# NILOIDE/A.I.gar

Hardware: AMD Instinct MI355X
Metric: env-steps/sec at 4096 bots x 100k pellets; 1/2/4/8 MI355X scaling (higher is better)
Workload: dtype f64; 1 GPU; C3: 4096 bots, 100000 pellets, 1152 viruses, split p=0.0025, eject p=0.01, field 4800, obs 854 floats/bot; start: data/c3_t50.npz (tick 50, mean cell mass 17.45, max 51.3) + 30 untimed random-policy ticks to settle; policy=random, parallelism=single-gpu

## Files before the change

aigar_amd/csrc/aigar_dev.h:

```cpp
#pragma once
#include <stdint.h>

#include "../../include/aigar.h"

namespace aigar {

#ifdef AIGAR_FLOOR
#ifdef AIGAR_FLOOR_OPAQUE
#define FLOOR(k) \
  if ((((AIGAR_FLOOR) >> (k)) & 1) && d.A > 0) return
#else
#define FLOOR(k) \
  if (((AIGAR_FLOOR) >> (k)) & 1) return
#endif
#else
#define FLOOR(k)
#endif

struct ArenaCtl {
  int64_t seq_next;
  int64_t tick;
  int64_t tick_sp;
  uint64_t key0, key1, ctr_pellet, ctr_virus;
  int64_t seq_base_upd;
// ... 31 lines not shown
  uint32_t pl_epoch;
  int pl_ticket;
  int n_pel_glob, n_eaten_glob, n_out, n_out_pel, n_undone, n_undone_glob;
  int n_ho;
  int n_ho_live;
  int n_cmd;
  int64_t stat[8];
};

enum : uint32_t {
  ERR_PELLET_CAP = 1, ERR_BLOB_CAP = 2, ERR_VIRUS_CAP = 4, ERR_EVENT_CAP = 8, ERR_WORK_CAP = 16,
  ERR_OBS_CAP = 32, ERR_CAND_CAP = 64, ERR_SLOT = 128, ERR_PIX_CAP = 256, ERR_TILE_CAP = 512, ERR_TILE_LOOKUP = 1024,
  ERR_TILE_OBS = 2048,
  ERR_TILE_PASSES = 4096,
  ERR_PREDICT = 8192,
  ERR_TILE_HANDOFF = 16384,
  ERR_CLAIM = 32768
};
enum : uint32_t { WARN_NEW_VIRUS_EATS = 1, WARN_DEAD_VIRUS = 2, WARN_TILE_OBS = 4 };
enum : uint32_t { DIRTY_VIRUS = 1, DIRTY_BLOB = 2 };

enum : uint32_t { PH_MERGE = 0, PH_VB = 1, PH_PV = 2, PH_PELLET = 3, PH_BLOB = 4, PH_PP = 5, PH_SPAWN = 6 };

struct TileRec {
  int32_t kind, idx;
  int64_t seq;
  double x, y;
};
enum : int32_t { TR_HDR = 0, TR_PELLET = 1, TR_BLOB = 2, TR_CELL = 3, TR_HIST = 4, TR_CMD = 5 };
constexpr int kHcapMax = 256;

struct alignas(32) PelRec {
// ... 38 lines not shown
  double *spec_x, *spec_y, *spec_m;
  double pow_n032[17];
  int cshift;
  int cshift_c;
  int Pcap, Ecap, Vcap, Wcap, EVcap;
  int PR;
  int PS;
  int PD;
  int PH1;
  int virus_enabled;
  double max_pellets, max_viruses;
  int G, L;
  uint32_t obs_ch, obs_ex;
  int flags;
  int pp_par;
  int share_cells;
  ArenaCtl *ctl;
  int *p_alive, *p_respawn, *p_ncells, *p_split, *p_eject, *p_pend;
  double *p_cmdx, *p_cmdy;
  double *p_fx, *p_fy, *p_fs, *p_mass;
  int *p_split_lh;
  uint8_t *p_role;
  int *p_time;
  double *o_last_mass;
  uint8_t *p_list;
  int *p_newc, *p_newb, *p_seqoff, *p_bloboff;
  int *p_heavy;
  double *c_x, *c_y, *c_m, *c_r, *c_vx, *c_vy, *c_svx, *c_svy, *c_mt;
  int *c_svc;
  uint32_t *c_flags;
  int64_t *c_seq;
// ... 70 lines not shown
```

aigar_amd/csrc/api.hip:

```cpp
#include <dlfcn.h>
#include <hip/hip_runtime.h>

#include <algorithm>
#include <cmath>
#include <cstdarg>
#include <cstdio>
#include <cstdlib>
#include <cstring>
#include <string>
#include <vector>

#include "../../include/aigar.h"
#include "aigar_dev.h"
#include "aigar_sem.h"

namespace aigar {
void launch_tick(const Dev &d, hipStream_t s, int rounds, int64_t *scr_k, int *scr_v,
                 const RandomPolicy *rp = nullptr);
void launch_tick_pre(const Dev &d, hipStream_t s, int64_t *scr_k, int *scr_v, const RandomPolicy *rp);
void launch_tick_post(const Dev &d, hipStream_t s, int64_t *scr_k, int *scr_v);
void launch_tile_pass(const Dev &d, hipStream_t s, int rounds, int64_t *scr_k, int *scr_v, int first);
void launch_tile_policy(const Dev &d, hipStream_t s, int greedy_split, uint8_t *mask, int cap);
void launch_tile_cmd_apply(const Dev &d, hipStream_t s, int box_recs);
void launch_pel_gather(const Dev &d, hipStream_t s, int a);
// ... 265 lines not shown
      cfg->obs_channels & (AIGAR_OBS_SELF_LF | AIGAR_OBS_SELF_SLF | AIGAR_OBS_ENEMY_LF | AIGAR_OBS_ENEMY_SLF))
    return fail("aigar_create: ALL_PLAYER_GRID with last-frame grids is undefined in the reference");
  if ((cfg->flags & AIGAR_FLAG_SCORE) &&
      (std::max(1, cfg->tile_x) * std::max(1, cfg->tile_y) > 1 || (cfg->tile_flags & AIGAR_TILE_FORCE)))
    return fail("aigar_create: AIGAR_FLAG_SCORE (the mass history score) is not kept on a tiled handle");
  int ndev = 0;
  HIPCHK(hipGetDeviceCount(&ndev));
  if (cfg->device < 0 || cfg->device >= ndev) return fail("aigar_create: device %d not present (%d devices)", cfg->device, ndev);
  HIPCHK(hipSetDevice(cfg->device));
  aigar_handle *h = new aigar_handle();
  h->cfg = *cfg;
  if (getenv("AIGAR_NO_GRAPH")) h->use_graph = false;
  if (const char *u = getenv("AIGAR_RUN_UNROLL")) h->run_unroll = std::max(1, std::min(64, atoi(u)));
  if (getenv("AIGAR_TILE_GRAPH")) h->tile_graph = true;
  h->d.pp_par = getenv("AIGAR_PP_SERIAL") ? 0 : 1;
  h->d.share_cells = 0;
  if (const char *r = getenv("AIGAR_FOOD_ROUNDS")) h->rounds = std::max(1, std::min(16, atoi(r)));
  Dev &d = h->d;
  d.A = cfg->n_arenas;
  d.B = cfg->bots_per_arena;
  d.NP = d.A * d.B;
  d.size = cfg->field_size > 0 ? cfg->field_size : (int)(75 * std::sqrt((double)d.B));
  d.cols = (int)std::ceil(d.size / 20.0);
  d.H = d.cols * d.cols;
  d.virus_enabled = cfg->virus_enabled ? 1 : 0;
  d.max_pellets = cfg->max_pellets >= 0 ? cfg->max_pellets : (double)d.size * d.size * 0.015;
  d.max_viruses = cfg->max_viruses >= 0 ? cfg->max_viruses : (double)d.size * d.size * 0.00005;
  if (!d.virus_enabled) d.max_viruses = 0;
  auto r64 = [](int v) { return (v + 63) / 64 * 64; };
  d.Ecap = r64(cfg->blob_cap > 0 ? cfg->blob_cap : 4 * d.B + 256);
  d.Pcap = r64(cfg->pellet_cap > 0 ? cfg->pellet_cap : (int)std::ceil(d.max_pellets) + d.Ecap + 64);
// ... 207 lines not shown
  free_all(h);
  delete h;
  return 0;
}

static int check_device_errors(aigar_handle *h) {
  std::vector<ArenaCtl> ctl(h->d.A);
  HIPCHK(hipMemcpyAsync(ctl.data(), h->d.ctl, sizeof(ArenaCtl) * h->d.A, hipMemcpyDeviceToHost, h->stream));
  HIPCHK(hipStreamSynchronize(h->stream));
  for (int a = 0; a < h->d.A; a++)
    if (ctl[a].err)
      return fail("device error bits 0x%x in arena %d (1 pellet cap, 2 blob cap, 4 virus cap, 8 event cap, "
                  "16 worklist cap, 32 observation cap, 64 candidate cap, 128 slot, 256 pixel-frame object cap, "
                  "512 tile message cap, 1024 tile record lookup, 2048 tile view beyond the held pellets, "
                  "4096 tiled tick ended with undone cells, 8192 new-cell / blob counts not as predicted, "
                  "16384 more dead bots to hand off than hand-off slots, 32768 cell claims left at the claim bound)",
                  ctl[a].err, a);
  return 0;
}

static size_t pix_hist_bytes(const aigar_handle *h) {
  return (h->pix.flags & AIGAR_PIX_LAST) ? sizeof(uint32_t) * h->d.NP * (size_t)h->pix.side * h->pix.side : 0;
}
__global__ void __launch_bounds__(256) k_pix_hist_clear_arenas(uint32_t *hist, size_t row, const int *al) {
  uint32_t *p = hist + (size_t)al[blockIdx.y] * row;
  for (size_t i = blockIdx.x * (size_t)blockDim.x + threadIdx.x; i < row; i += (size_t)gridDim.x * blockDim.x) p[i] = 0;
}
__global__ void __launch_bounds__(256) k_pix_hist_clear_bots(uint32_t *hist, size_t LL, size_t n, const uint8_t *mask) {
  const size_t i = blockIdx.x * (size_t)blockDim.x + threadIdx.x;
  if (i < n && (!mask || mask[i / LL])) hist[i] = 0;
}
// ... 159 lines not shown
    else launch_tick(h->d, h->stream, rounds, h->scr_k, h->scr_v);
  }
  HIPCHK(hipGetLastError());
  return 0;
}

static void launch_env_step(aigar_handle *h, hipStream_t s, const aigar_run_params &p, void *out, int dtype,
                            bool policy_done = false, bool fuse_next = false) {
#ifdef AIGAR_NO_POLICY_FOLD
  const RandomPolicy rp{0, 0, 0, 0};
  if (p.policy == AIGAR_POLICY_RANDOM) launch_policy(h->d, s, p.p_split, p.p_eject, p.seed);
#else
  const RandomPolicy rp{p.policy == AIGAR_POLICY_RANDOM, p.p_split, p.p_eject, p.seed};
#endif
  if (p.policy == AIGAR_POLICY_GREEDY && !policy_done) launch_policy_greedy(h->d, s, p.greedy_split ? 1 : 0, nullptr, -1);
  Dev dt = h->d;
  dt.share_cells = p.policy == AIGAR_POLICY_GREEDY ? 1 : 0;
  launch_tick(dt, s, food_rounds(h), h->scr_k, h->scr_v, &rp);
  if (out) launch_observe(h->d, s, out, dtype, 0, nullptr, fuse_next ? (p.greedy_split ? 1 : 0) : -1);
}
static bool run_fuses_greedy(const aigar_handle *h, const aigar_run_params &p, const void *out) {
  return p.policy == AIGAR_POLICY_GREEDY && out && observe_fuses_greedy(h->d) &&
         !getenv("AIGAR_NO_GREEDY_FUSE");
}

extern "C" int aigar_run(aigar_handle *h, int n_steps, const aigar_run_params *p, void *obs_out, int dtype) {
  if (!h || !p) return fail("null argument");
  if (n_steps < 0) return fail("n_steps < 0");
  if (p->policy < AIGAR_POLICY_NONE || p->policy > AIGAR_POLICY_GREEDY) return fail("unknown policy %d", p->policy);
  if (obs_out && dtype != 0 && dtype != 1) return fail("dtype must be 0 (float64) or 1 (float32)");
  HIPCHK(hipSetDevice(h->cfg.device));
  if (h->d.flags & AIGAR_FLAG_EVENTS)
    hipLaunchKernelGGL(k_step_begin, dim3((h->d.A + 63) / 64), dim3(64), 0, h->stream, h->d);
// ... 1325 lines not shown
```

aigar_amd/csrc/tick.hip:

```cpp
#include <hip/hip_runtime.h>

#include "aigar_dev.h"
#include "aigar_sem.h"
#include "aigar_wave.h"

namespace aigar {

#define GTID ((int)(blockIdx.x * blockDim.x + threadIdx.x))
#define TILE_GATE(d)                                          \
  do {                                                        \
    if ((d).tile_gate && (d).ctl[0].n_undone_glob == 0) return; \
  } while (0)

#ifdef AIGAR_PHASE_TIMING
constexpr int kPtWaves = 8192;
__device__ unsigned int g_ptw[9][kPtWaves][8];
__device__ unsigned int g_ptid[9][kPtWaves][2];
__device__ __forceinline__ void pt_ids(unsigned *o) {
  unsigned a, b;
  asm volatile("s_getreg_b32 %0, hwreg(HW_REG_HW_ID)" : "=s"(a));
  asm volatile("s_getreg_b32 %0, hwreg(HW_REG_XCC_ID)" : "=s"(b));
  o[0] = a;
  o[1] = b;
}
// ... 1233 lines not shown
  __syncthreads();
}
__device__ __forceinline__ int cgrid_cols(const Dev &d) { return (d.cols + (1 << d.cshift_c) - 1) >> d.cshift_c; }
__device__ __forceinline__ int cgrid_bucket(const Dev &d, double x, double y) {
  const int sh = d.cshift_c;
  return (center_bucket_coord(y, d.cols) >> sh) * cgrid_cols(d) + (center_bucket_coord(x, d.cols) >> sh);
}
__device__ __forceinline__ int *cgrid_counts(const Dev &d, int a, int row) {
  return d.cgcnt + ((size_t)a * 2 + row) * CG_STRIDE;
}
__device__ __forceinline__ void cgrid_count_cell(const Dev &d, int a, size_t ci, double x, double y) {
  const int per = kMaxCells * d.B, slot = (int)(ci / d.NP), p = (int)(ci - (size_t)slot * d.NP) - a * d.B;
  const int b = cgrid_bucket(d, x, y);
  d.c_rank[(size_t)a * per + (size_t)slot * d.B + p] = (b << 17) | atomicAdd(&cgrid_counts(d, a, 0)[b], 1);
}
__device__ void count_scan_256(int *cnt, int n, int *start, int *lds, uint16_t *bits) {
  __shared__ int wsum[4];
  const int tid = threadIdx.x, lane = tid & 63, w = tid >> 6;
  const int4 *c4 = reinterpret_cast<const int4 *>(cnt);
  int v[16], sum = 0;
#pragma unroll
  for (int k = 0; k < 4; k++) {
    const int j = tid * 16 + 4 * k;
    int4 q = j < n ? c4[j >> 2] : make_int4(0, 0, 0, 0);
    v[4 * k] = j < n ? q.x : 0;
    v[4 * k + 1] = j + 1 < n ? q.y : 0;
    v[4 * k + 2] = j + 2 < n ? q.z : 0;
    v[4 * k + 3] = j + 3 < n ? q.w : 0;
  }
#pragma unroll
  for (int k = 0; k < 16; k++) sum += v[k];
  if (bits) {
    uint32_t bm = 0;
#pragma unroll
    for (int k = 0; k < 16; k++) bm |= (v[k] != 0 ? 1u : 0u) << k;
    bits[tid] = (uint16_t)bm;
  }
  int inc = sum;
#pragma unroll
  for (int off = 1; off < 64; off <<= 1) {
    int t = __shfl_up(inc, off);
    if (lane >= off) inc += t;
  }
  if (lane == 63) wsum[w] = inc;
  __syncthreads();
  int run = inc - sum;
  for (int k = 0; k < w; k++) run += wsum[k];
  const int total = wsum[0] + wsum[1] + wsum[2] + wsum[3];
#pragma unroll
  for (int k = 0; k < 16; k++) {
    const int j = tid * 16 + k;
    if (j < n) {
      start[j] = run;
      if (lds) lds[j] = run;
      cnt[j] = 0;
    }
    run += v[k];
  }
  if (tid == 0) {
    start[n] = total;
    if (lds) lds[n] = total;
  }
}
__device__ void cgrid_scan_block(const Dev &d, int a) {
  const int cc = cgrid_cols(d);
  count_scan_256(cgrid_counts(d, a, 0), cc * cc, d.cstart + (size_t)a * (d.H + 1), nullptr, nullptr);
}
__device__ __forceinline__ void cgrid_place_player(const Dev &d, int gp, int n) {
  const int NP = d.NP, a = gp / d.B, p = gp - a * d.B, per = kMaxCells * d.B;
  const int *start = d.cstart + (size_t)a * (d.H + 1);
  int *items = d.citems + (size_t)a * per;
  for (int k = 0; k < n; k++) {
    const int slot = d.p_list[k * NP + gp];
    const int br = d.c_rank[(size_t)a * per + (size_t)slot * d.B + p];
    items[start[br >> 17] + (br & 0x1FFFF)] = slot * NP + gp;
  }
}


__device__ __forceinline__ int prow_entry(const Dev &d, int bx, int by) { return by * (d.cols + 1) + bx; }
__device__ __forceinline__ void prow_count(const Dev &d, int a, int j) {
// ... 195 lines not shown
  const int *st = d.vstart + (size_t)a * (d.H + 1);
  const int *it = d.vitems + (size_t)a * d.Vcap;
  const int nv = c.n_vir;
  grid_visit(st, it, d.cols, qb, expand_for(c.rmax_virus), [&](int i) {
    const size_t g = (size_t)a * d.Vcap + i;
    if (i >= nv || !(d.v_flags[g] & F_ALIVE)) return;
    const double vx = d.v_x[g], vy = d.v_y[g], vr = d.v_r[g];
    if (!rect_hit(footprint(vx, vy, vr, d.size), qb)) return;
    if (!overlap(vx, vy, d.v_m[g], vr, bx, by, bm, br)) return;
    if (atomicExch(&d.v_active[g], 1) != 0) return;
    const int w = atomicAdd(&d.ctl[a].n_pend, 1);
    if (w < d.Wcap) d.work[(size_t)a * d.Wcap + w] = i;
    else set_err(d, a, ERR_WORK_CAP);
  }, d.cshift);
}
__device__ void count_scan_256(int *cnt, int n, int *start, int *lds, uint16_t *bits);
__device__ void blob_grid_place(const Dev &d, int a, int *cnt) {
  const int tid = threadIdx.x, T = blockDim.x, s = d.cshift;
  const int cc = (d.cols + (1 << s) - 1) >> s;
  const int n = d.ctl[a].n_blob;
  int *items = d.bitems + (size_t)a * d.Ecap;
  const int *rank = d.b_rank + (size_t)a * d.Ecap;
  count_scan_256(cgrid_counts(d, a, 1), cc * cc, d.bstart + (size_t)a * (d.H + 1), cnt,
                 reinterpret_cast<uint16_t *>(d.bmap + (size_t)a * 64));
  __syncthreads();
  if (tid == 0) d.ctl[a].n_blob_live = cnt[cc * cc];
  for (int i = tid; i < n; i += T) {
    const int rk = rank[i];
    if (rk < 0) continue;
    const int b = rk >> 12, r = rk & 4095;
    if (r == 4095) set_err(d, a, ERR_SLOT);
// ... 475 lines not shown

__device__ __forceinline__ void wave_sync_lds() {
  __builtin_amdgcn_fence(__ATOMIC_RELEASE, "wavefront");
  __builtin_amdgcn_wave_barrier();
  __builtin_amdgcn_fence(__ATOMIC_ACQUIRE, "wavefront");
}
__device__ __forceinline__ double wave_sum(double v) {
#pragma unroll
  for (int off = 32; off > 0; off >>= 1) v += __shfl_xor(v, off);
  return v;
}

constexpr int PREP_CAND = 128;
constexpr int PREP_WAVES = 1;
__device__ __forceinline__ double tile_rall() { return sqrt(kMaxMass / kPi) * (1 + 1e-9); }
template <bool SHARE>
__global__ void __launch_bounds__(256, 4) k_food_prep(Dev d, int rounds, int resume) {
  FLOOR(4);
  TILE_GATE(d);
  __shared__ int64_t s_seq[4][PREP_CAND];
  __shared__ double s_x[4][PREP_CAND], s_y[4][PREP_CAND], s_m[4][PREP_CAND];
  __shared__ int s_idx[4][PREP_CAND];
  __shared__ uint8_t s_sel[4][PREP_CAND];
  __shared__ uint64_t s_bm[4][64];
  if (!resume && (int)blockIdx.x < d.A) cgrid_scan_block(d, blockIdx.x);
  PT_BEGIN(0);
  const int w = threadIdx.x >> 6, lane = threadIdx.x & 63;
  const int wi = xcd_block(blockIdx.x, gridDim.x) * 4 + w, gp = wi / PREP_WAVES,
            h = wi - gp * PREP_WAVES;
  static_assert(PREP_WAVES == 1, "the block's cell sharing assumes one wave per player");
  __shared__ int q_n[4], q_next[4], q_a[4];
  if constexpr (SHARE) {
    if (lane == 0) {
      q_n[w] = 0;
      q_next[w] = 1;
    }
    __syncthreads();
  }
  if (gp < d.NP && gp % d.B == 0 && h == 0 && lane == 0) d.ctl[gp / d.B].food_undone[1] = 0;
  if (gp >= d.NP) return;
  const int s_first = uni((int)d.p_list[h * d.NP + gp]);
  s_bm[w][lane] = d.bmap[(size_t)(gp / d.B) * 64 + lane];
  const bool alive = d.p_alive[gp];
  const int NP = d.NP, a = gp / d.B;
  Food F(d, a);
  const uint32_t base = d.ctl[a].food_round;
  const int n0 = uni(d.p_ncells[gp]);
  const int n = alive ? n0 : 0;
  if (SHARE && lane == 0) {
    q_a[w] = a;
    __hip_atomic_store(&q_n[w], n, __ATOMIC_RELAXED, __HIP_MEMORY_SCOPE_WORKGROUP);
  }
  PT_MARK(0, 1);
  auto prep_cell = [&](const int gpc, const int k, const size_t ci) {
    const int p = gpc - a * d.B;
    uint32_t prio = (uint32_t)p * kMaxCells + k;
    const size_t kc = (size_t)k * NP + gpc;
    if (resume && d.f_done[ci] == 1) return;
    double x = uni(d.c_x[ci]), y = uni(d.c_y[ci]), m = uni(d.c_m[ci]), r = uni(d.c_r[ci]);
    int64_t cseq = uni(d.c_seq[ci]);
    PT_MARK(0, 2);
    Rect q = uni(footprint(x, y, r, d.size));
    if (d.tiled && !tile_near_rect(d, rect_grow(footprint(x, y, fmax(r, tile_rall()), d.size), 1, d.cols), 2)) {
      if (lane == 0) {
        d.f_cnt[kc] = 0;
        d.f_done[ci] = 2;
      }
// ... 120 lines not shown
      if (i < cnt && s_sel[w][i]) {
        int64_t sq = s_seq[w][i];
        int rk = 0;
        for (int jj = 0; jj < cnt; jj++) rk += (s_sel[w][jj] && s_seq[w][jj] < sq);
        lst[rk] = s_idx[w][i];
        atomicMax((unsigned long long *)F.owner(s_idx[w][i]), (unsigned long long)key);
      }
    }
    if (lane == 0) {
      d.f_cnt[kc] = (uint8_t)nsel;
      d.f_done[ci] = (nsel == 0);
    }
    wave_sync_lds();
    PT_MARK(0, 6);
  };
  if constexpr (!SHARE) {
    for (int k = 0; k < n; k++) prep_cell(gp, k, (size_t)(k == 0 ? s_first : uni((int)d.p_list[k * NP + gp])) * NP + gp);
    return;
  }
  const int g0 = xcd_block(blockIdx.x, gridDim.x) * 4;
  int gpc = gp, kc = n > 0 ? 0 : -1, sc = s_first;
  int step = 0;
  for (; step <= 4 * kMaxCells; step++) {
    if (kc < 0) {
      for (int t = 0; t < 4 && kc < 0; t++) {
        const int w2 = (w + t) & 3;
        const int n2 = __builtin_amdgcn_readfirstlane(__hip_atomic_load(&q_n[w2], __ATOMIC_RELAXED, __HIP_MEMORY_SCOPE_WORKGROUP));
        if (n2 <= 1 || __builtin_amdgcn_readfirstlane(q_a[w2]) != a) continue;
        const int leader = __ffsll((long long)__ballot(1)) - 1;
        int k = 0;
        if (lane == leader) k = atomicAdd(&q_next[w2], 1);
        k = __builtin_amdgcn_readlane(k, leader);
        if (k >= n2) continue;
        gpc = __builtin_amdgcn_readfirstlane(g0 + w2);
        kc = k;
        sc = __builtin_amdgcn_readfirstlane((int)d.p_list[k * NP + gpc]);
      }
      if (kc < 0) break;
    }
    prep_cell(gpc, kc, (size_t)sc * NP + gpc);
    kc = -1;
  }
  if (step > 4 * kMaxCells && lane == wave_leader()) set_err(d, a, ERR_CLAIM);
}
__device__ __forceinline__ void food_eat(const Dev &d, const Food &F, int a, int j, uint32_t prio, int t,
                                         int64_t cseq, int64_t fseq, double fm, double &m, double &r, int &eaten,
                                         bool own, double fx, double fy) {
  const bool bl = Food::blob(j);
  if (own) {
    ev_push(d, a, bl ? PH_BLOB : PH_PELLET, ((uint64_t)prio << 16) | (uint64_t)t, bl ? 7 : 6, cseq, fseq);
    if (d.tiled) {
      if (bl) tile_out(d, TR_BLOB, j & ~kBlobBit, fseq, 0.0, 0.0);
      else tile_out(d, TR_PELLET, 0, fseq, fx, fy);
    }
  }
  m = grow_mass(m, fm);
  r = radius_of(m);
  F.kill(j);
// ... 454 lines not shown
      if (lane == 0) occ[wd] = bits;
#endif
    }
  }
#if AIGAR_OCC_BATCH
  if (q0 >= 0) flush();
#endif
}

__device__ __forceinline__ void pp_active_own(const Dev &d PT_PARAMS) {
  const int lane = threadIdx.x & 63;
  const int gp = xcd_block(blockIdx.x, gridDim.x) * 4 + (threadIdx.x >> 6);
  if (d.tiled && gp == 0 && lane == 0 && d.ctl[0].n_undone_glob != 0) atomicOr(&d.ctl[0].err, ERR_TILE_PASSES);
  if (gp >= d.NP) return;
  const int s_first = d.p_list[gp];
  if (!d.p_alive[gp]) return;
  const int NP = d.NP, a = gp / d.B;
  const int *st = d.cstart + (size_t)a * (d.H + 1);
  const int *it = d.citems + (size_t)a * kMaxCells * d.B;
  int E = expand_for(d.ctl[a].rmax_cell);
  int n = d.p_ncells[gp];
  bool anyp = false;
  PT_MARK(3, 1);
  for (int k = 0; k < n; k++) {
    size_t ci = (size_t)(k == 0 ? s_first : d.p_list[k * NP + gp]) * NP + gp;
    double x = d.c_x[ci], y = d.c_y[ci], m = d.c_m[ci], r = d.c_r[ci];
    PT_MARK(3, 2);
    Rect q = footprint(x, y, r, d.size);
    occ_add(d, a, q);
    bool any = wave_any_in_grid(st, it, d.cols, q, E, [&](int e) {
      if (!(d.c_flags[e] & F_ALIVE) || (int)(e % NP) <= gp) return false;
      if (!rect_hit(cell_rect(d, e), q)) return false;
      double me = d.c_m[e];
      return overlap(x, y, m, r, d.c_x[e], d.c_y[e], me, d.c_r[e]) && (can_eat(m, me) || can_eat(me, m));
    }, d.cshift_c);
    if (lane == 0) d.c_active[ci] = any;
    anyp |= any;
    PT_MARK(3, 3);
  }
  if (anyp && lane == 0) {
    int w = atomicAdd(&d.ctl[a].n_pend, 1);
    if (w < d.Wcap) d.work[(size_t)a * d.Wcap + w] = gp - a * d.B;
    else set_err(d, a, ERR_WORK_CAP);
  }
}
template <bool SHARE>
__global__ void __launch_bounds__(256) k_pp_active(Dev d) {
  FLOOR(6);
  PT_BEGIN(3);
  if constexpr (!SHARE) {
    pp_active_own(d PT_ARGS);
    return;
  }
  const int lane = threadIdx.x & 63, w = threadIdx.x >> 6;
  const int g0 = xcd_block(blockIdx.x, gridDim.x) * 4, gp = g0 + w;
  __shared__ int q_n[4], q_next[4], q_done[4], q_any[4], q_a[4];
  if (lane == 0) {
    q_n[w] = 0;
    q_next[w] = 1;
    q_done[w] = 0;
    q_any[w] = 0;
  }
  __syncthreads();
  if (d.tiled && gp == 0 && lane == 0 && d.ctl[0].n_undone_glob != 0) atomicOr(&d.ctl[0].err, ERR_TILE_PASSES);
  if (gp >= d.NP) return;
  const int s_first = d.p_list[gp];
  const bool alive = d.p_alive[gp];
  const int NP = d.NP, a = gp / d.B;
  const int *st = d.cstart + (size_t)a * (d.H + 1);
  const int *it = d.citems + (size_t)a * kMaxCells * d.B;
  const int E = expand_for(d.ctl[a].rmax_cell);
  const int n = alive ? d.p_ncells[gp] : 0;
  if (lane == 0) {
    q_a[w] = a;
    __hip_atomic_store(&q_n[w], n, __ATOMIC_RELAXED, __HIP_MEMORY_SCOPE_WORKGROUP);
  }
  PT_MARK(3, 1);
  int wc = w, kc = n > 0 ? 0 : -1, nc = n, sc = s_first;
  int step = 0;
  for (; step <= 4 * kMaxCells; step++) {
    if (kc < 0) {
      for (int t = 0; t < 4 && kc < 0; t++) {
        const int w2 = (w + t) & 3;
        const int n2 = __builtin_amdgcn_readfirstlane(__hip_atomic_load(&q_n[w2], __ATOMIC_RELAXED, __HIP_MEMORY_SCOPE_WORKGROUP));
        if (n2 <= 1 || __builtin_amdgcn_readfirstlane(q_a[w2]) != a) continue;
        const int leader = __ffsll((long long)__ballot(1)) - 1;
        int k = 0;
        if (lane == leader) k = atomicAdd(&q_next[w2], 1);
        k = __builtin_amdgcn_readlane(k, leader);
        if (k >= n2) continue;
        wc = w2;
        kc = k;
        nc = n2;
        sc = __builtin_amdgcn_readfirstlane((int)d.p_list[k * NP + g0 + w2]);
      }
      if (kc < 0) break;
    }
    const int gpc = __builtin_amdgcn_readfirstlane(g0 + wc);
    const size_t ci = (size_t)sc * NP + gpc;
    double x = d.c_x[ci], y = d.c_y[ci], m = d.c_m[ci], r = d.c_r[ci];
    PT_MARK(3, 2);
    Rect q = footprint(x, y, r, d.size);
    occ_add(d, a, q);
    bool any = wave_any_in_grid(st, it, d.cols, q, E, [&](int e) {
      if (!(d.c_flags[e] & F_ALIVE) || (int)(e % NP) <= gpc) return false;
      if (!rect_hit(cell_rect(d, e), q)) return false;
      double me = d.c_m[e];
      return overlap(x, y, m, r, d.c_x[e], d.c_y[e], me, d.c_r[e]) && (can_eat(m, me) || can_eat(me, m));
    }, d.cshift_c);
    const int leader = __ffsll((long long)__ballot(1)) - 1;
    if (lane == leader) {
      d.c_active[ci] = any;
      bool push = any;
      if (nc > 1) {
        if (any) atomicOr(&q_any[wc], 1);
        push = atomicAdd(&q_done[wc], 1) == nc - 1 &&
               __hip_atomic_load(&q_any[wc], __ATOMIC_RELAXED, __HIP_MEMORY_SCOPE_WORKGROUP) != 0;
      }
      if (push) {
        const int wq = atomicAdd(&d.ctl[a].n_pend, 1);
        if (wq < d.Wcap) d.work[(size_t)a * d.Wcap + wq] = gpc - a * d.B;
        else set_err(d, a, ERR_WORK_CAP);
      }
    }
    PT_MARK(3, 3);
    kc = -1;
  }
  if (step > 4 * kMaxCells && lane == wave_leader()) set_err(d, a, ERR_CLAIM);
}

__device__ __forceinline__ bool remove_cell(const Dev &d, int a, size_t e, uint64_t &order, bool writer = true) {
  const int NP = d.NP;
  int gp = (int)(e % NP);
  uint8_t slot = (uint8_t)(e / NP);
  uint8_t l[kMaxCells];
#pragma unroll
  for (int k = 0; k < kMaxCells; k++) l[k] = d.p_list[k * NP + gp];
  const int n = d.p_ncells[gp];
  d.c_flags[e] = 0;
  int w = 0;
#pragma unroll
  for (int k = 0; k < kMaxCells; k++)
    if (k < n && l[k] != slot) d.p_list[(w++) * NP + gp] = l[k];
// ... 1539 lines not shown
  int64_t *k;
  int *v;
};

void launch_pellet_rows(const Dev &d, hipStream_t s) {
  const long n = (long)d.A * d.Pcap;
  hipLaunchKernelGGL(k_prow_count, dim3(nblk(n, 256)), dim3(256), 0, s, d);
  hipLaunchKernelGGL(k_prow_scan, dim3(d.cols, d.A), dim3(256), 0, s, d);
  hipLaunchKernelGGL(k_prow_scatter, dim3(nblk(n, 256)), dim3(256), 0, s, d);
}


static void launch_food(const Dev &d, hipStream_t s, int rounds, Scratch scr, int resume = 0, int fold = 0) {
  rounds = std::max(rounds, 1);
  const int g = nblk(d.NP, 256);
  if (d.share_cells)
    hipLaunchKernelGGL(k_food_prep<true>, dim3(std::max(nblk((long)d.NP * PREP_WAVES, 4), resume ? 0 : d.A)), dim3(256),
                       0, s, d, rounds, resume);
  else
    hipLaunchKernelGGL(k_food_prep<false>, dim3(std::max(nblk((long)d.NP * PREP_WAVES, 4), resume ? 0 : d.A)), dim3(256),
                       0, s, d, rounds, resume);
  for (int r = 1; r <= rounds; r++) {
    hipLaunchKernelGGL(k_food_commit, dim3(g), dim3(256), 0, s, d, r, r == rounds ? 1 : 0, scr.k, scr.v, rounds,
                       fold && r == rounds ? 1 : 0, r == 1 && !resume ? 1 : 0);
  }
  if (!fold) hipLaunchKernelGGL(k_food_serial, dim3(d.A), dim3(64), 0, s, d, scr.k, scr.v, rounds);
}

void launch_player_fov(const Dev &d, hipStream_t s);
void launch_tick_pre(const Dev &d, hipStream_t s, int64_t *scr_k, int *scr_v, const RandomPolicy *rp) {
  hipLaunchKernelGGL(k_players, dim3(d.pl_tiles + 1 + (d.Ecap + kPlT - 1) / kPlT, d.A), dim3(kPlT), 0, s, d, rp ? *rp : RandomPolicy{0, 0, 0, 0});
  if (d.virus_enabled)
    hipLaunchKernelGGL(k_merge_pv, dim3(nblk(d.NP, 256) + nblk((long)d.A * d.Ecap, 256) + d.A), dim3(256), 0, s, d,
                       scr_k, scr_v);
  else
    hipLaunchKernelGGL(k_merge_vb, dim3(nblk(d.NP, 256) + d.A), dim3(256), 0, s, d, scr_k, scr_v, 0);
}
void launch_tick_post(const Dev &d, hipStream_t s, int64_t *scr_k, int *scr_v) {
  if (d.share_cells) hipLaunchKernelGGL(k_pp_active<true>, dim3(nblk(d.NP, 4)), dim3(256), 0, s, d);
  else hipLaunchKernelGGL(k_pp_active<false>, dim3(nblk(d.NP, 4)), dim3(256), 0, s, d);
  hipLaunchKernelGGL(k_spawn_plan, dim3(d.A), dim3(1024),
                     sizeof(uint32_t) * ((d.B + 31) / 32) * PPG_WAVES + (d.B <= PP_LOWN_MAX ? sizeof(int) * d.B : 0), s, d, 0,
                     scr_k, scr_v, 1, 1);
  const int nbF = nblk(d.NP, 256);
  const int nbV = d.virus_enabled ? nblk((long)d.A * d.Vcap, 256) : 0;
  hipLaunchKernelGGL(k_pel_update, dim3(d.A * d.cols + nbF + nbV), dim3(256), 0, s, d, nbF);
}
void launch_score_sample(const Dev &d, hipStream_t s);
void launch_tick(const Dev &d, hipStream_t s, int rounds, int64_t *scr_k, int *scr_v, const RandomPolicy *rp) {
  if (d.sc) launch_score_sample(d, s);
  launch_tick_pre(d, s, scr_k, scr_v, rp);
  launch_food(d, s, rounds, Scratch{scr_k, scr_v}, 0, 1);
  launch_tick_post(d, s, scr_k, scr_v);
}

// ... 320 lines not shown
```

Measured before the change: 47.36 million env-steps/s.

## Process all of a player's cells in one wave pass for food prep and pp-active

Replaces the greedy-only cross-wave cell-sharing scheme (workgroup claim queues) with single-wave multi-cell paths in k_food_prep and pp_active_own. These split the 64 lanes across a player's cells, gather grid rows and candidates for all cells with wave prefix sums, and fall back to the per-cell loop when a cap is exceeded. The head blocks also overlap the cell-grid count scan with prefetching the first cell's data, using a raw s_barrier. This targets serial per-cell loops for multi-cell players under the random policy, at the cost of more shuffle and ballot work and higher register pressure.

```diff
diff --git a/aigar_amd/csrc/aigar_dev.h b/aigar_amd/csrc/aigar_dev.h
--- a/aigar_amd/csrc/aigar_dev.h
+++ b/aigar_amd/csrc/aigar_dev.h
@@ -69,8 +69,7 @@
   ERR_TILE_OBS = 2048,
   ERR_TILE_PASSES = 4096,
   ERR_PREDICT = 8192,
-  ERR_TILE_HANDOFF = 16384,
-  ERR_CLAIM = 32768
+  ERR_TILE_HANDOFF = 16384
 };
 enum : uint32_t { WARN_NEW_VIRUS_EATS = 1, WARN_DEAD_VIRUS = 2, WARN_TILE_OBS = 4 };
 enum : uint32_t { DIRTY_VIRUS = 1, DIRTY_BLOB = 2 };
@@ -139,7 +138,6 @@
   uint32_t obs_ch, obs_ex;
   int flags;
   int pp_par;
-  int share_cells;
   ArenaCtl *ctl;
   int *p_alive, *p_respawn, *p_ncells, *p_split, *p_eject, *p_pend;
   double *p_cmdx, *p_cmdy;
diff --git a/aigar_amd/csrc/api.hip b/aigar_amd/csrc/api.hip
--- a/aigar_amd/csrc/api.hip
+++ b/aigar_amd/csrc/api.hip
@@ -303,7 +303,6 @@
   if (const char *u = getenv("AIGAR_RUN_UNROLL")) h->run_unroll = std::max(1, std::min(64, atoi(u)));
   if (getenv("AIGAR_TILE_GRAPH")) h->tile_graph = true;
   h->d.pp_par = getenv("AIGAR_PP_SERIAL") ? 0 : 1;
-  h->d.share_cells = 0;
   if (const char *r = getenv("AIGAR_FOOD_ROUNDS")) h->rounds = std::max(1, std::min(16, atoi(r)));
   Dev &d = h->d;
   d.A = cfg->n_arenas;
@@ -541,7 +540,7 @@
                   "16 worklist cap, 32 observation cap, 64 candidate cap, 128 slot, 256 pixel-frame object cap, "
                   "512 tile message cap, 1024 tile record lookup, 2048 tile view beyond the held pellets, "
                   "4096 tiled tick ended with undone cells, 8192 new-cell / blob counts not as predicted, "
-                  "16384 more dead bots to hand off than hand-off slots, 32768 cell claims left at the claim bound)",
+                  "16384 more dead bots to hand off than hand-off slots)",
                   ctl[a].err, a);
   return 0;
 }
@@ -731,9 +730,7 @@
   const RandomPolicy rp{p.policy == AIGAR_POLICY_RANDOM, p.p_split, p.p_eject, p.seed};
 #endif
   if (p.policy == AIGAR_POLICY_GREEDY && !policy_done) launch_policy_greedy(h->d, s, p.greedy_split ? 1 : 0, nullptr, -1);
-  Dev dt = h->d;
-  dt.share_cells = p.policy == AIGAR_POLICY_GREEDY ? 1 : 0;
-  launch_tick(dt, s, food_rounds(h), h->scr_k, h->scr_v, &rp);
+  launch_tick(h->d, s, food_rounds(h), h->scr_k, h->scr_v, &rp);
   if (out) launch_observe(h->d, s, out, dtype, 0, nullptr, fuse_next ? (p.greedy_split ? 1 : 0) : -1);
 }
 static bool run_fuses_greedy(const aigar_handle *h, const aigar_run_params &p, const void *out) {
diff --git a/aigar_amd/csrc/tick.hip b/aigar_amd/csrc/tick.hip
--- a/aigar_amd/csrc/tick.hip
+++ b/aigar_amd/csrc/tick.hip
@@ -1271,15 +1271,26 @@
   const int b = cgrid_bucket(d, x, y);
   d.c_rank[(size_t)a * per + (size_t)slot * d.B + p] = (b << 17) | atomicAdd(&cgrid_counts(d, a, 0)[b], 1);
 }
-__device__ void count_scan_256(int *cnt, int n, int *start, int *lds, uint16_t *bits) {
+struct NoMid {
+  __device__ void operator()() const {}
+};
+template <class Mid = NoMid>
+__device__ void count_scan_256(int *cnt, int n, int *start, int *lds, uint16_t *bits, Mid mid = Mid()) {
   __shared__ int wsum[4];
   const int tid = threadIdx.x, lane = tid & 63, w = tid >> 6;
   const int4 *c4 = reinterpret_cast<const int4 *>(cnt);
   int v[16], sum = 0;
+  int4 q4[4];
 #pragma unroll
   for (int k = 0; k < 4; k++) {
     const int j = tid * 16 + 4 * k;
-    int4 q = j < n ? c4[j >> 2] : make_int4(0, 0, 0, 0);
+    q4[k] = j < n ? c4[j >> 2] : make_int4(0, 0, 0, 0);
+  }
+  mid();
+#pragma unroll
+  for (int k = 0; k < 4; k++) {
+    const int j = tid * 16 + 4 * k;
+    const int4 q = q4[k];
     v[4 * k] = j < n ? q.x : 0;
     v[4 * k + 1] = j + 1 < n ? q.y : 0;
     v[4 * k + 2] = j + 2 < n ? q.z : 0;
@@ -1300,7 +1311,13 @@
     if (lane >= off) inc += t;
   }
   if (lane == 63) wsum[w] = inc;
-  __syncthreads();
+  if constexpr (std::is_same<Mid, NoMid>::value) {
+    __syncthreads();
+  } else {
+    __builtin_amdgcn_fence(__ATOMIC_RELEASE, "workgroup", "local");
+    __builtin_amdgcn_s_barrier();
+    __builtin_amdgcn_fence(__ATOMIC_ACQUIRE, "workgroup", "local");
+  }
   int run = inc - sum;
   for (int k = 0; k < w; k++) run += wsum[k];
   const int total = wsum[0] + wsum[1] + wsum[2] + wsum[3];
@@ -1319,9 +1336,10 @@
     if (lds) lds[n] = total;
   }
 }
-__device__ void cgrid_scan_block(const Dev &d, int a) {
+template <class Mid = NoMid>
+__device__ __forceinline__ void cgrid_scan_block(const Dev &d, int a, Mid mid = Mid()) {
   const int cc = cgrid_cols(d);
-  count_scan_256(cgrid_counts(d, a, 0), cc * cc, d.cstart + (size_t)a * (d.H + 1), nullptr, nullptr);
+  count_scan_256(cgrid_counts(d, a, 0), cc * cc, d.cstart + (size_t)a * (d.H + 1), nullptr, nullptr, mid);
 }
 __device__ __forceinline__ void cgrid_place_player(const Dev &d, int gp, int n) {
   const int NP = d.NP, a = gp / d.B, p = gp - a * d.B, per = kMaxCells * d.B;
@@ -1547,7 +1565,6 @@
     else set_err(d, a, ERR_WORK_CAP);
   }, d.cshift);
 }
-__device__ void count_scan_256(int *cnt, int n, int *start, int *lds, uint16_t *bits);
 __device__ void blob_grid_place(const Dev &d, int a, int *cnt) {
   const int tid = threadIdx.x, T = blockDim.x, s = d.cshift;
   const int cc = (d.cols + (1 << s) - 1) >> s;
@@ -2053,7 +2070,6 @@
 constexpr int PREP_CAND = 128;
 constexpr int PREP_WAVES = 1;
 __device__ __forceinline__ double tile_rall() { return sqrt(kMaxMass / kPi) * (1 + 1e-9); }
-template <bool SHARE>
 __global__ void __launch_bounds__(256, 4) k_food_prep(Dev d, int rounds, int resume) {
   FLOOR(4);
   TILE_GATE(d);
@@ -2062,34 +2078,42 @@
   __shared__ int s_idx[4][PREP_CAND];
   __shared__ uint8_t s_sel[4][PREP_CAND];
   __shared__ uint64_t s_bm[4][64];
-  if (!resume && (int)blockIdx.x < d.A) cgrid_scan_block(d, blockIdx.x);
+  const bool head = !resume && (int)blockIdx.x < d.A;
   PT_BEGIN(0);
   const int w = threadIdx.x >> 6, lane = threadIdx.x & 63;
   const int wi = xcd_block(blockIdx.x, gridDim.x) * 4 + w, gp = wi / PREP_WAVES,
             h = wi - gp * PREP_WAVES;
-  static_assert(PREP_WAVES == 1, "the block's cell sharing assumes one wave per player");
-  __shared__ int q_n[4], q_next[4], q_a[4];
-  if constexpr (SHARE) {
-    if (lane == 0) {
-      q_n[w] = 0;
-      q_next[w] = 1;
-    }
-    __syncthreads();
-  }
+  static_assert(PREP_WAVES == 1, "prep_multi assumes one wave per player");
   if (gp < d.NP && gp % d.B == 0 && h == 0 && lane == 0) d.ctl[gp / d.B].food_undone[1] = 0;
-  if (gp >= d.NP) return;
-  const int s_first = uni((int)d.p_list[h * d.NP + gp]);
-  s_bm[w][lane] = d.bmap[(size_t)(gp / d.B) * 64 + lane];
-  const bool alive = d.p_alive[gp];
-  const int NP = d.NP, a = gp / d.B;
+  if (gp >= d.NP && !head) return;
+  const int gpl = min(gp, d.NP - 1);
+  const int NP = d.NP, a = gpl / d.B;
+  const int v_first = d.p_list[h * NP + gpl];
+  const int v_slot = d.p_list[(lane < kMaxCells ? lane : 0) * NP + gpl];
+  s_bm[w][lane] = d.bmap[(size_t)a * 64 + lane];
+  const bool alive = d.p_alive[gpl];
   Food F(d, a);
   const uint32_t base = d.ctl[a].food_round;
-  const int n0 = uni(d.p_ncells[gp]);
+  const int v_n = d.p_ncells[gpl];
+  if (head) {
+    double t0 = 0, t1 = 0, t2 = 0, t3 = 0;
+    long long t4 = 0;
+    cgrid_scan_block(d, blockIdx.x, [&] {
+      if (gp < NP && alive && v_n > 0) {
+        const size_t ci = (size_t)v_first * NP + gp;
+        t0 = d.c_x[ci];
+        t1 = d.c_y[ci];
+        t2 = d.c_m[ci];
+        t3 = d.c_r[ci];
+        t4 = d.c_seq[ci];
+      }
+    });
+    asm volatile("" ::"v"(t0), "v"(t1), "v"(t2), "v"(t3), "v"(t4));
+    if (gp >= NP) return;
+  }
+  const int s_first = uni(v_first);
+  const int n0 = uni(v_n);
   const int n = alive ? n0 : 0;
-  if (SHARE && lane == 0) {
-    q_a[w] = a;
-    __hip_atomic_store(&q_n[w], n, __ATOMIC_RELAXED, __HIP_MEMORY_SCOPE_WORKGROUP);
-  }
   PT_MARK(0, 1);
   auto prep_cell = [&](const int gpc, const int k, const size_t ci) {
     const int p = gpc - a * d.B;
@@ -2240,34 +2264,148 @@
     wave_sync_lds();
     PT_MARK(0, 6);
   };
-  if constexpr (!SHARE) {
-    for (int k = 0; k < n; k++) prep_cell(gp, k, (size_t)(k == 0 ? s_first : uni((int)d.p_list[k * NP + gp])) * NP + gp);
-    return;
-  }
-  const int g0 = xcd_block(blockIdx.x, gridDim.x) * 4;
-  int gpc = gp, kc = n > 0 ? 0 : -1, sc = s_first;
-  int step = 0;
-  for (; step <= 4 * kMaxCells; step++) {
-    if (kc < 0) {
-      for (int t = 0; t < 4 && kc < 0; t++) {
-        const int w2 = (w + t) & 3;
-        const int n2 = __builtin_amdgcn_readfirstlane(__hip_atomic_load(&q_n[w2], __ATOMIC_RELAXED, __HIP_MEMORY_SCOPE_WORKGROUP));
-        if (n2 <= 1 || __builtin_amdgcn_readfirstlane(q_a[w2]) != a) continue;
-        const int leader = __ffsll((long long)__ballot(1)) - 1;
-        int k = 0;
-        if (lane == leader) k = atomicAdd(&q_next[w2], 1);
-        k = __builtin_amdgcn_readlane(k, leader);
-        if (k >= n2) continue;
-        gpc = __builtin_amdgcn_readfirstlane(g0 + w2);
-        kc = k;
-        sc = __builtin_amdgcn_readfirstlane((int)d.p_list[k * NP + gpc]);
-      }
-      if (kc < 0) break;
-    }
-    prep_cell(gpc, kc, (size_t)sc * NP + gpc);
-    kc = -1;
-  }
-  if (step > 4 * kMaxCells && lane == wave_leader()) set_err(d, a, ERR_CLAIM);
+  auto prep_multi = [&]() -> bool {
+    const int n = uni(n0);
+    const int g = lane >> 2, sub = lane & 3;
+    const bool has = g < n;
+    const int slot = __shfl(v_slot, g);
+    const size_t ci = (size_t)(has ? slot : s_first) * NP + gp;
+    const double x = d.c_x[ci], y = d.c_y[ci], m = d.c_m[ci], r = d.c_r[ci];
+    PT_MARK(0, 2);
+    const Rect q = footprint(x, y, r, d.size);
+    const Span sp = grid_span(q, 1, d.cols, 0);
+    const int ngrid = sp.by1 - sp.by0 + 1;
+    const bool qok = has && q.x0 <= q.x1 && q.y0 <= q.y1;
+    auto prefix = [&](int v, int &total) {
+      int inc = v;
+#pragma unroll
+      for (int off = 1; off < 64; off <<= 1) {
+        const int t = __shfl_up(inc, off);
+        if (lane >= off) inc += t;
+      }
+      total = uni(__shfl(inc, 63));
+      return inc - v;
+    };
+    int R;
+    const int rbase = prefix(qok && sub == 0 ? ngrid + (F.nst > 0 ? 1 : 0) : 0, R);
+    if (R > 64) return false;
+    int c = 0;
+    for (int k = 1; k < n; k++) c = (__builtin_amdgcn_readlane(rbase, 4 * k) <= lane) ? k : c;
+    const int rr = lane - __shfl(rbase, 4 * c), c_by0 = __shfl(sp.by0, 4 * c), c_bx0 = __shfl(sp.bx0, 4 * c),
+              c_bx1 = __shfl(sp.bx1, 4 * c), c_ng = __shfl(ngrid, 4 * c);
+    int lo = 0, len = 0;
+    if (lane < R) {
+      if (rr < c_ng) {
+        const int *st = d.pstart + (size_t)a * d.PH1;
+        const int b = (c_by0 + rr) * (d.cols + 1);
+        lo = st[b + c_bx0];
+        len = st[b + c_bx1 + 1] - lo;
+      } else {
+        lo = F.n0;
+        len = F.nst;
+      }
+    }
+    int T;
+    const int excl = prefix(len, T);
+    int cnt = 0, pc = 0;
+    for (int t0 = 0; t0 < T; t0 += 64) {
+      const int t = t0 + lane;
+      int row = 0;
+      for (int k = 1; k < R; k++) row = (__builtin_amdgcn_readlane(excl, k) <= t) ? k : row;
+      const int j = __shfl(lo, row) + (t - __shfl(excl, row)), cc = __shfl(c, row);
+      const Rect qc{__shfl(q.x0, 4 * cc), __shfl(q.x1, 4 * cc), __shfl(q.y0, 4 * cc), __shfl(q.y1, 4 * cc)};
+      bool keep = false;
+      double fx = 0, fy = 0, fm = 0;
+      int64_t fsq = 0;
+      if (t < T) {
+        F.load(j, fx, fy, fm, fsq);
+        keep = rect_hit(footprint(fx, fy, pellet_radius(fm), d.size), qc);
+      }
+      const unsigned long long bal = __ballot(keep);
+      const int at = cnt + __popcll(bal & ((1ull << lane) - 1));
+      if (keep && at < PREP_CAND) {
+        s_seq[w][at] = Food::order_key(j, fsq);
+        s_x[w][at] = fx;
+        s_y[w][at] = fy;
+        s_m[w][at] = fm;
+        s_idx[w][at] = j;
+        s_sel[w][at] = (uint8_t)cc;
+      }
+      cnt += __popcll(bal);
+      for (int k = 0; k < n; k++) {
+        const int ck = __popcll(__ballot(keep && cc == k));
+        pc += g == k ? ck : 0;
+      }
+    }
+    PT_MARK(0, 3);
+    if (cnt > PREP_CAND) return false;
+    int all;
+    const int ps = __shfl(prefix(sub == 0 ? pc : 0, all), lane & ~3);
+    wave_sync_lds();
+    double ls = 0;
+    for (int i = sub; i < pc; i += 4) ls += s_m[w][ps + i];
+    ls += __shfl_xor(ls, 1);
+    ls += __shfl_xor(ls, 2);
+    const double M = py_min(kMaxMass, (m + ls) * (1 + 1e-9));
+    const double Rm = fmax(r, radius_of(M)) * (1 + 1e-9);
+    bool near = false;
+    const Rect qb = footprint(x, y, Rm, d.size);
+    if (has && F.any_blobs() && qb.x0 <= qb.x1 && qb.y0 <= qb.y1) {
+      const Span gb = grid_span(qb, 1, d.cols, d.cshift);
+      const int bw = gb.bx1 - gb.bx0 + 1, nb = bw * (gb.by1 - gb.by0 + 1);
+      for (int i = sub; i < nb; i += 4) {
+        const int b = (gb.by0 + i / bw) * gb.stride + gb.bx0 + i % bw;
+        near |= (s_bm[w][b >> 6] >> (b & 63)) & 1;
+      }
+    }
+    if (__ballot(near)) return false;
+    PT_MARK(0, 4);
+    int nsel = 0;
+    for (int i0 = 0; i0 < cnt; i0 += 64) {
+      const int i = i0 + lane;
+      const int cc = i < cnt ? s_sel[w][i] : 0;
+      const double cx = __shfl(x, 4 * cc), cy = __shfl(y, 4 * cc), cM = __shfl(M, 4 * cc), cR = __shfl(Rm, 4 * cc);
+      bool sel = false;
+      if (i < cnt) {
+        const double fx = s_x[w][i], fy = s_y[w][i];
+        sel = (cM > 1.25 * s_m[w][i]) && ((cx - fx) * (cx - fx) + (cy - fy) * (cy - fy) < cR * cR);
+      }
+      for (int k = 0; k < n; k++) {
+        const int ck = __popcll(__ballot(sel && cc == k));
+        nsel += g == k ? ck : 0;
+      }
+      if (sel) s_sel[w][i] = (uint8_t)(cc | 0x80);
+    }
+    if (__ballot(has && nsel > FCAP)) return false;
+    wave_sync_lds();
+    PT_MARK(0, 5);
+    const int p = gp - a * d.B;
+    for (int i0 = 0; i0 < cnt; i0 += 64) {
+      const int i = i0 + lane;
+      const int tag = i < cnt ? s_sel[w][i] : 0, cc = tag & 0x7F;
+      const int cps = __shfl(ps, 4 * cc), cpc = __shfl(pc, 4 * cc);
+      if (tag & 0x80) {
+        const int64_t sq = s_seq[w][i];
+        int rk = 0;
+        for (int jj = cps; jj < cps + cpc; jj++) rk += ((s_sel[w][jj] & 0x80) && s_seq[w][jj] < sq);
+        const int j = s_idx[w][i];
+        d.f_list[((size_t)cc * NP + gp) * FCAP + rk] = j;
+        atomicMax((unsigned long long *)F.owner(j),
+                  (unsigned long long)food_key(base + 1, (uint32_t)p * kMaxCells + cc));
+      }
+    }
+    if (has && sub == 0) {
+      d.f_cnt[(size_t)g * NP + gp] = (uint8_t)nsel;
+      d.f_done[ci] = (nsel == 0);
+    }
+    PT_MARK(0, 6);
+    return true;
+  };
+  if (n >= 2 && !resume && !d.tiled) {
+    if (prep_multi()) return;
+    wave_sync_lds();
+  }
+  for (int k = 0; k < n; k++) prep_cell(gp, k, (size_t)(k == 0 ? s_first : uni((int)d.p_list[k * NP + gp])) * NP + gp);
 }
 __device__ __forceinline__ void food_eat(const Dev &d, const Food &F, int a, int j, uint32_t prio, int t,
                                          int64_t cseq, int64_t fseq, double fm, double &m, double &r, int &eaten,
@@ -2752,6 +2890,7 @@
   if (d.tiled && gp == 0 && lane == 0 && d.ctl[0].n_undone_glob != 0) atomicOr(&d.ctl[0].err, ERR_TILE_PASSES);
   if (gp >= d.NP) return;
   const int s_first = d.p_list[gp];
+  const int v_slot = d.p_list[(lane < kMaxCells ? lane : 0) * d.NP + gp];
   if (!d.p_alive[gp]) return;
   const int NP = d.NP, a = gp / d.B;
   const int *st = d.cstart + (size_t)a * (d.H + 1);
@@ -2760,6 +2899,67 @@
   int n = d.p_ncells[gp];
   bool anyp = false;
   PT_MARK(3, 1);
+  auto pp_multi = [&]() -> bool {
+    const int nu = uni(n);
+    const bool has = lane < nu;
+    const size_t ci = (size_t)(has ? v_slot : s_first) * NP + gp;
+    const double x = d.c_x[ci], y = d.c_y[ci], m = d.c_m[ci], r = d.c_r[ci];
+    PT_MARK(3, 2);
+    const Rect q = footprint(x, y, r, d.size);
+    const Span sp = grid_span(q, E, d.cols, d.cshift_c);
+    const int nrow = has && q.x0 <= q.x1 && q.y0 <= q.y1 ? sp.by1 - sp.by0 + 1 : 0;
+    auto prefix = [&](int v, int &total) {
+      int inc = v;
+#pragma unroll
+      for (int off = 1; off < 64; off <<= 1) {
+        const int t = __shfl_up(inc, off);
+        if (lane >= off) inc += t;
+      }
+      total = uni(__shfl(inc, 63));
+      return inc - v;
+    };
+    int R;
+    const int rbase = prefix(nrow, R);
+    if (R > 64) return false;
+    int c = 0;
+    for (int k = 1; k < nu; k++) c = (__builtin_amdgcn_readlane(rbase, k) <= lane) ? k : c;
+    const int rr = lane - __shfl(rbase, c), c_by0 = __shfl(sp.by0, c), c_bx0 = __shfl(sp.bx0, c),
+              c_bx1 = __shfl(sp.bx1, c);
+    int lo = 0, len = 0;
+    if (lane < R) {
+      const int b = (c_by0 + rr) * sp.stride;
+      lo = st[b + c_bx0];
+      len = st[b + c_bx1 + 1] - lo;
+    }
+    int T;
+    const int excl = prefix(len, T);
+    unsigned act = 0;
+    for (int t0 = 0; t0 < T && act != (1u << nu) - 1; t0 += 64) {
+      const int t = t0 + lane;
+      int row = 0;
+      for (int k = 1; k < R; k++) row = (__builtin_amdgcn_readlane(excl, k) <= t) ? k : row;
+      const int idx = __shfl(lo, row) + (t - __shfl(excl, row)), cc = __shfl(c, row);
+      const double cx = __shfl(x, cc), cy = __shfl(y, cc), cm = __shfl(m, cc), cr = __shfl(r, cc);
+      const Rect qc{__shfl(q.x0, cc), __shfl(q.x1, cc), __shfl(q.y0, cc), __shfl(q.y1, cc)};
+      bool hit = false;
+      if (t < T) {
+        const int e = it[idx];
+        if ((d.c_flags[e] & F_ALIVE) && (int)(e % NP) > gp && rect_hit(cell_rect(d, e), qc)) {
+          const double me = d.c_m[e];
+          hit = overlap(cx, cy, cm, cr, d.c_x[e], d.c_y[e], me, d.c_r[e]) && (can_eat(cm, me) || can_eat(me, cm));
+        }
+      }
+      for (int k = 0; k < nu; k++) act |= __ballot(hit && cc == k) ? 1u << k : 0u;
+    }
+    for (int k = 0; k < nu; k++)
+      occ_add(d, a, Rect{__builtin_amdgcn_readlane(q.x0, k), __builtin_amdgcn_readlane(q.x1, k),
+                         __builtin_amdgcn_readlane(q.y0, k), __builtin_amdgcn_readlane(q.y1, k)});
+    if (has) d.c_active[ci] = (act >> lane) & 1;
+    anyp = act != 0;
+    PT_MARK(3, 3);
+    return true;
+  };
+  if (n >= 2 && pp_multi()) n = 0;
   for (int k = 0; k < n; k++) {
     size_t ci = (size_t)(k == 0 ? s_first : d.p_list[k * NP + gp]) * NP + gp;
     double x = d.c_x[ci], y = d.c_y[ci], m = d.c_m[ci], r = d.c_r[ci];
@@ -2782,89 +2982,10 @@
     else set_err(d, a, ERR_WORK_CAP);
   }
 }
-template <bool SHARE>
 __global__ void __launch_bounds__(256) k_pp_active(Dev d) {
   FLOOR(6);
   PT_BEGIN(3);
-  if constexpr (!SHARE) {
-    pp_active_own(d PT_ARGS);
-    return;
-  }
-  const int lane = threadIdx.x & 63, w = threadIdx.x >> 6;
-  const int g0 = xcd_block(blockIdx.x, gridDim.x) * 4, gp = g0 + w;
-  __shared__ int q_n[4], q_next[4], q_done[4], q_any[4], q_a[4];
-  if (lane == 0) {
-    q_n[w] = 0;
-    q_next[w] = 1;
-    q_done[w] = 0;
-    q_any[w] = 0;
-  }
-  __syncthreads();
-  if (d.tiled && gp == 0 && lane == 0 && d.ctl[0].n_undone_glob != 0) atomicOr(&d.ctl[0].err, ERR_TILE_PASSES);
-  if (gp >= d.NP) return;
-  const int s_first = d.p_list[gp];
-  const bool alive = d.p_alive[gp];
-  const int NP = d.NP, a = gp / d.B;
-  const int *st = d.cstart + (size_t)a * (d.H + 1);
-  const int *it = d.citems + (size_t)a * kMaxCells * d.B;
-  const int E = expand_for(d.ctl[a].rmax_cell);
-  const int n = alive ? d.p_ncells[gp] : 0;
-  if (lane == 0) {
-    q_a[w] = a;
-    __hip_atomic_store(&q_n[w], n, __ATOMIC_RELAXED, __HIP_MEMORY_SCOPE_WORKGROUP);
-  }
-  PT_MARK(3, 1);
-  int wc = w, kc = n > 0 ? 0 : -1, nc = n, sc = s_first;
-  int step = 0;
-  for (; step <= 4 * kMaxCells; step++) {
-    if (kc < 0) {
-      for (int t = 0; t < 4 && kc < 0; t++) {
-        const int w2 = (w + t) & 3;
-        const int n2 = __builtin_amdgcn_readfirstlane(__hip_atomic_load(&q_n[w2], __ATOMIC_RELAXED, __HIP_MEMORY_SCOPE_WORKGROUP));
-        if (n2 <= 1 || __builtin_amdgcn_readfirstlane(q_a[w2]) != a) continue;
-        const int leader = __ffsll((long long)__ballot(1)) - 1;
-        int k = 0;
-        if (lane == leader) k = atomicAdd(&q_next[w2], 1);
-        k = __builtin_amdgcn_readlane(k, leader);
-        if (k >= n2) continue;
-        wc = w2;
-        kc = k;
-        nc = n2;
-        sc = __builtin_amdgcn_readfirstlane((int)d.p_list[k * NP + g0 + w2]);
-      }
-      if (kc < 0) break;
-    }
-    const int gpc = __builtin_amdgcn_readfirstlane(g0 + wc);
-    const size_t ci = (size_t)sc * NP + gpc;
-    double x = d.c_x[ci], y = d.c_y[ci], m = d.c_m[ci], r = d.c_r[ci];
-    PT_MARK(3, 2);
-    Rect q = footprint(x, y, r, d.size);
-    occ_add(d, a, q);
-    bool any = wave_any_in_grid(st, it, d.cols, q, E, [&](int e) {
-      if (!(d.c_flags[e] & F_ALIVE) || (int)(e % NP) <= gpc) return false;
-      if (!rect_hit(cell_rect(d, e), q)) return false;
-      double me = d.c_m[e];
-      return overlap(x, y, m, r, d.c_x[e], d.c_y[e], me, d.c_r[e]) && (can_eat(m, me) || can_eat(me, m));
-    }, d.cshift_c);
-    const int leader = __ffsll((long long)__ballot(1)) - 1;
-    if (lane == leader) {
-      d.c_active[ci] = any;
-      bool push = any;
-      if (nc > 1) {
-        if (any) atomicOr(&q_any[wc], 1);
-        push = atomicAdd(&q_done[wc], 1) == nc - 1 &&
-               __hip_atomic_load(&q_any[wc], __ATOMIC_RELAXED, __HIP_MEMORY_SCOPE_WORKGROUP) != 0;
-      }
-      if (push) {
-        const int wq = atomicAdd(&d.ctl[a].n_pend, 1);
-        if (wq < d.Wcap) d.work[(size_t)a * d.Wcap + wq] = gpc - a * d.B;
-        else set_err(d, a, ERR_WORK_CAP);
-      }
-    }
-    PT_MARK(3, 3);
-    kc = -1;
-  }
-  if (step > 4 * kMaxCells && lane == wave_leader()) set_err(d, a, ERR_CLAIM);
+  pp_active_own(d PT_ARGS);
 }
 
 __device__ __forceinline__ bool remove_cell(const Dev &d, int a, size_t e, uint64_t &order, bool writer = true) {
@@ -4434,12 +4555,8 @@
 static void launch_food(const Dev &d, hipStream_t s, int rounds, Scratch scr, int resume = 0, int fold = 0) {
   rounds = std::max(rounds, 1);
   const int g = nblk(d.NP, 256);
-  if (d.share_cells)
-    hipLaunchKernelGGL(k_food_prep<true>, dim3(std::max(nblk((long)d.NP * PREP_WAVES, 4), resume ? 0 : d.A)), dim3(256),
-                       0, s, d, rounds, resume);
-  else
-    hipLaunchKernelGGL(k_food_prep<false>, dim3(std::max(nblk((long)d.NP * PREP_WAVES, 4), resume ? 0 : d.A)), dim3(256),
-                       0, s, d, rounds, resume);
+  hipLaunchKernelGGL(k_food_prep, dim3(std::max(nblk((long)d.NP * PREP_WAVES, 4), resume ? 0 : d.A)), dim3(256), 0, s, d,
+                     rounds, resume);
   for (int r = 1; r <= rounds; r++) {
     hipLaunchKernelGGL(k_food_commit, dim3(g), dim3(256), 0, s, d, r, r == rounds ? 1 : 0, scr.k, scr.v, rounds,
                        fold && r == rounds ? 1 : 0, r == 1 && !resume ? 1 : 0);
@@ -4457,8 +4574,7 @@
     hipLaunchKernelGGL(k_merge_vb, dim3(nblk(d.NP, 256) + d.A), dim3(256), 0, s, d, scr_k, scr_v, 0);
 }
 void launch_tick_post(const Dev &d, hipStream_t s, int64_t *scr_k, int *scr_v) {
-  if (d.share_cells) hipLaunchKernelGGL(k_pp_active<true>, dim3(nblk(d.NP, 4)), dim3(256), 0, s, d);
-  else hipLaunchKernelGGL(k_pp_active<false>, dim3(nblk(d.NP, 4)), dim3(256), 0, s, d);
+  hipLaunchKernelGGL(k_pp_active, dim3(nblk(d.NP, 4)), dim3(256), 0, s, d);
   hipLaunchKernelGGL(k_spawn_plan, dim3(d.A), dim3(1024),
                      sizeof(uint32_t) * ((d.B + 31) / 32) * PPG_WAVES + (d.B <= PP_LOWN_MAX ? sizeof(int) * d.B : 0), s, d, 0,
                      scr_k, scr_v, 1, 1);
```

Measured after the change: 47.89 million env-steps/s (median of 6 runs). 1.01x the previous value.
